# muzishen/IMAGHarmony

Hardware: AMD Instinct MI355X
Metric: 1024^2 SDXL images/sec (30 DDIM steps, PNS N seeds) (higher is better)
Workload: dtype bf16

## Files before the change

### imagharmony_amd/csrc/elementwise.hip

```cpp
#include <algorithm>

#include "imh_common.h"
#include "imh_kernels.h"
#include "imh_philox.h"

namespace imh {

enum : int { EW_TIMESTEP = 0, EW_SILU = 1, EW_CONCAT = 2, EW_CONV_IN = 3, EW_CFG_STEP = 4, EW_CAST_F32 = 5,
             EW_ADD = 6, EW_STEP_SET = 7, EW_CFG_RESCALE = 8, EW_SOFTMAX = 9, EW_ROW_STATS = 10, EW_STEP_ROW = 11, EW_GATHER_ROWS = 12,
             EW_CFG_MSTEP = 13 };

template <typename T>
__global__ void timestep_kernel(const EwParams p) {
    const int dim = p.i0, half = dim >> 1;
    const long long total = p.n * half;
    for (long long i = (long long)blockIdx.x * blockDim.x + threadIdx.x; i < total; i += (long long)gridDim.x * blockDim.x) {
        const int v = (int)(i / half), j = (int)(i % half);
        const float t = p.step ? ((const float*)p.a)[*p.step] : ((const float*)p.a)[v];
        const float f = expf(-9.210340371976184f * (float)j / (float)half);
        const float a = t * f;
        T* y = (T*)p.y + (size_t)v * dim;
        y[j] = from_f32<T>(cosf(a));
        y[half + j] = from_f32<T>(sinf(a));
    }
}

template <typename T>
__global__ void silu_kernel(const EwParams p) {
    typedef typename Vec<T>::v8 v8;
    const long long nv = p.n >> 3;
    for (long long i = (long long)blockIdx.x * blockDim.x + threadIdx.x; i < nv; i += (long long)gridDim.x * blockDim.x) {
        v8 v = ((const v8*)p.a)[i], o;
#pragma unroll
        for (int e = 0; e < 8; ++e) o[e] = from_f32<T>(silu_f(to_f32(v[e])));
        ((v8*)p.y)[i] = o;
    }
}

template <typename T>
__global__ void add_kernel(const EwParams p) {
    typedef typename Vec<T>::v8 v8;
    const long long nv = p.n >> 3;
    for (long long i = (long long)blockIdx.x * blockDim.x + threadIdx.x; i < nv; i += (long long)gridDim.x * blockDim.x) {
        v8 u = ((const v8*)p.a)[i], v = ((const v8*)p.b)[i], o;
#pragma unroll
        for (int e = 0; e < 8; ++e) o[e] = from_f32<T>(to_f32(u[e]) + to_f32(v[e]));
        ((v8*)p.y)[i] = o;
    }
}

template <typename T>
__global__ void concat_kernel(const EwParams p) {
    typedef typename Vec<T>::v8 v8;
    const int c1 = p.i0 >> 3, c2 = p.i1 >> 3, ct = c1 + c2;
    const long long total = p.n * ct;
    for (long long i = (long long)blockIdx.x * blockDim.x + threadIdx.x; i < total; i += (long long)gridDim.x * blockDim.x) {
        const long long pix = i / ct;
        const int c = (int)(i - pix * ct);
        v8 v = c < c1 ? ((const v8*)p.a)[pix * c1 + c] : ((const v8*)p.b)[pix * c2 + (c - c1)];
        ((v8*)p.y)[i] = v;
    }
}

template <typename T, int CIN>
__global__ __launch_bounds__(CIN > 4 ? 512 : 256) void conv_in_kernel(const EwParams p) {
    typedef typename Vec<T>::v8 v8;
    constexpr int KT = CIN * 9;
    extern __shared__ float wl[];
    const int S = p.i0, H = p.i1, W = p.i2, C0 = p.i3, Bout = p.i4;
    const T* w = (const T*)p.w;
    for (int co = threadIdx.x; co < C0; co += blockDim.x) {
#pragma unroll
        for (int k = 0; k < KT; ++k) wl[k * C0 + co] = to_f32(w[co * KT + k]);
    }
    for (int i = threadIdx.x; i < C0; i += blockDim.x) wl[KT * C0 + i] = p.bias ? to_f32(((const T*)p.bias)[i]) : 0.f;
    __syncthreads();
    const int cg = C0 >> 3;
    const float in_scale = p.tab ? p.tab[*p.step] : p.f0;
    const long long total = (long long)Bout * H * W * 8;
    const float* lat = (const float*)p.a;
    for (long long i = (long long)blockIdx.x * blockDim.x + threadIdx.x; i < total; i += (long long)gridDim.x * blockDim.x) {
        const int l8 = (int)(i & 7);
        const long long pix = i >> 3;
        const int x = (int)(pix % W);
        const int y = (int)((pix / W) % H);
        const int b = (int)(pix / ((long long)W * H));
        const float* src = lat + (size_t)(b % S) * 4 * H * W;
        float tap[KT];
#pragma unroll
        for (int ci = 0; ci < 4; ++ci)
#pragma unroll
            for (int ky = 0; ky < 3; ++ky)
#pragma unroll
                for (int kx = 0; kx < 3; ++kx) {
                    const int iy = y + ky - 1, ix = x + kx - 1;
                    const bool in = iy >= 0 && iy < H && ix >= 0 && ix < W;
                    const float v = in ? src[((size_t)ci * H + iy) * W + ix] * in_scale : 0.f;
                    tap[ci * 9 + ky * 3 + kx] = to_f32(from_f32<T>(v));
                }
        if constexpr (CIN > 4) {
            const float* src2 = p.x2 + (size_t)(b % S) * (CIN - 4) * H * W;
#pragma unroll
            for (int ci = 4; ci < CIN; ++ci)
#pragma unroll
                for (int ky = 0; ky < 3; ++ky)
#pragma unroll
                    for (int kx = 0; kx < 3; ++kx) {
                        const int iy = y + ky - 1, ix = x + kx - 1;
                        const bool in = iy >= 0 && iy < H && ix >= 0 && ix < W;
                        const float v = in ? src2[((size_t)(ci - 4) * H + iy) * W + ix] : 0.f;
                        tap[ci * 9 + ky * 3 + kx] = to_f32(from_f32<T>(v));
                    }
        }
        for (int c8 = l8; c8 < cg; c8 += 8) {
            float acc[8];
#pragma unroll
            for (int e = 0; e < 8; ++e) acc[e] = wl[KT * C0 + c8 * 8 + e];
#pragma unroll
            for (int k = 0; k < KT; ++k) {
                const float* wr = wl + k * C0 + c8 * 8;
#pragma unroll
                for (int e = 0; e < 8; ++e) acc[e] += tap[k] * wr[e];
            }
            v8 o;
#pragma unroll
            for (int e = 0; e < 8; ++e) o[e] = from_f32<T>(acc[e]);
            ((v8*)p.y)[pix * cg + c8] = o;
        }
    }
}

template <typename T, bool BLEND>
__global__ void cfg_step_kernel(const EwParams p) {
    const int S = p.i0, HW = p.i1;
    const long long total = (long long)S * HW * 4;
    const T* np_ = (const T*)p.a;
    float* lat = (float*)p.y;
    const float cx = p.tab ? p.tab[*p.step * 2] : p.f0;
    const float ce = p.tab ? p.tab[*p.step * 2 + 1] : p.f1;
    float ba = 0.f, bb = 0.f;
    if constexpr (BLEND) { ba = p.blend_tab[*p.step * 2]; bb = p.blend_tab[*p.step * 2 + 1]; }
    for (long long i = (long long)blockIdx.x * blockDim.x + threadIdx.x; i < total; i += (long long)gridDim.x * blockDim.x) {
        const int pix = (int)(i % HW);
        const int ch = (int)((i / HW) % 4);
        const int s = (int)(i / ((long long)HW * 4));
        if (!BLEND || np_) {
            float eps;
            if (p.i3) {
                const float u = to_f32(np_[((size_t)s * HW + pix) * 4 + ch]);
                const float c = to_f32(np_[((size_t)(S + s) * HW + pix) * 4 + ch]);
                eps = u + p.f2 * (c - u);
            } else {
                eps = to_f32(np_[((size_t)s * HW + pix) * 4 + ch]);
            }
            if (p.w) eps *= ((const float*)p.w)[s];
            if (p.b) ((float*)p.b)[i] = eps;
            lat[i] = cx * lat[i] + ce * eps;
        }
        if constexpr (BLEND) {
            const float m = p.mask[(size_t)(s % p.i4) * HW + pix];
            const float pv = ba * p.x2[i] + bb * p.noise[i];
            lat[i] = (1.0f - m) * pv + m * lat[i];
        }
    }
}

template <typename T, bool BLEND, bool SEEDED = false>
__global__ void cfg_mstep_kernel(const EwParams p) {
    const int S = p.i0, HW = p.i1;
    const long long total = (long long)S * HW * 4;
    const T* np_ = (const T*)p.a;
    float* lat = (float*)p.y;
    float* hist = (float*)p.b;
    const int row = *p.step;
    const float* c = p.tab + (size_t)row * 6;
    const float cx = c[0], ce = c[1], ch = c[2], cn = c[3], hx = c[4], he = c[5];
    const float* z = p.bias ? (const float*)p.bias + (size_t)row * (size_t)total : nullptr;
    float ba = 0.f, bb = 0.f;
    if constexpr (BLEND) { ba = p.blend_tab[row * 2]; bb = p.blend_tab[row * 2 + 1]; }
    if constexpr (SEEDED) {
        const bool gen = cn != 0.f;
        const long long quads = (long long)S * HW;
        for (long long q = (long long)blockIdx.x * blockDim.x + threadIdx.x; q < quads; q += (long long)gridDim.x * blockDim.x) {
            const int s = (int)(q / HW);
            PhiloxNormals zn = {{0.f, 0.f, 0.f, 0.f}};
            if (gen) zn = seeded_normals(p.seeds + (size_t)s * 4, (uint32_t)(q - (long long)s * HW), (uint32_t)row, p.noise_stream);
#pragma unroll
            for (int k = 0; k < 4; ++k) {
                const long long i = q * 4 + k;
                const int pix = (int)(i % HW);
                const int chn = (int)((i / HW) % 4);
                float eps;
                if (p.i3) {
                    const float u = to_f32(np_[((size_t)s * HW + pix) * 4 + chn]);
                    const float cnd = to_f32(np_[((size_t)(S + s) * HW + pix) * 4 + chn]);
                    eps = u + p.f2 * (cnd - u);
                } else {
                    eps = to_f32(np_[((size_t)s * HW + pix) * 4 + chn]);
                }
                if (p.w) eps *= ((const float*)p.w)[s];
                const float x = lat[i];
                float y = cx * x + ce * eps;
                if (hist) {
                    y += ch * hist[i];
                    hist[i] = hx * x + he * eps;
                }
                if (gen) y += cn * zn.z[k];
                if constexpr (BLEND) {
                    const float m = p.mask[(size_t)(s % p.i4) * HW + pix];
                    const float pv = ba * p.x2[i] + bb * p.noise[i];
                    y = (1.0f - m) * pv + m * y;
                }
                lat[i] = y;
            }
        }
        return;
    }
    for (long long i = (long long)blockIdx.x * blockDim.x + threadIdx.x; i < total; i += (long long)gridDim.x * blockDim.x) {
        const int pix = (int)(i % HW);
        const int chn = (int)((i / HW) % 4);
        const int s = (int)(i / ((long long)HW * 4));
        float eps;
        if (p.i3) {
            const float u = to_f32(np_[((size_t)s * HW + pix) * 4 + chn]);
            const float cnd = to_f32(np_[((size_t)(S + s) * HW + pix) * 4 + chn]);
            eps = u + p.f2 * (cnd - u);
        } else {
            eps = to_f32(np_[((size_t)s * HW + pix) * 4 + chn]);
        }
        if (p.w) eps *= ((const float*)p.w)[s];
        const float x = lat[i];
        float y = cx * x + ce * eps;
        if (hist) {
            y += ch * hist[i];
            hist[i] = hx * x + he * eps;
        }
        if (z) y += cn * z[i];
        if constexpr (BLEND) {
            const float m = p.mask[(size_t)(s % p.i4) * HW + pix];
            const float pv = ba * p.x2[i] + bb * p.noise[i];
            y = (1.0f - m) * pv + m * y;
        }
        lat[i] = y;
    }
}

__global__ void randn_seeded_kernel(const RandnParams p) {
    const int HW = p.HW;
    const uint32_t row = p.step ? (uint32_t)*p.step : p.row;
    const long long quads = (long long)p.S * HW;
    for (long long q = (long long)blockIdx.x * blockDim.x + threadIdx.x; q < quads; q += (long long)gridDim.x * blockDim.x) {
        const int s = (int)(q / HW);
        const uint32_t qs = p.quad0 + (uint32_t)(q - (long long)s * HW);
        if (p.raw) {
            const PhiloxWords w = seeded_words(p.seeds + (size_t)s * 4, qs, row, p.noise_stream);
            uint32_t* y = (uint32_t*)p.y + q * 4;
#pragma unroll
            for (int k = 0; k < 4; ++k) y[k] = w.w[k];
        } else {
            const PhiloxNormals n = seeded_normals(p.seeds + (size_t)s * 4, qs, row, p.noise_stream);
            float* y = (float*)p.y + q * 4;
#pragma unroll
            for (int k = 0; k < 4; ++k) y[k] = n.z[k];
        }
    }
}

template <typename T>
__global__ __launch_bounds__(256) void cfg_rescale_kernel(const EwParams p) {
    __shared__ double red[4][256];
    const int S = p.i0, HW = p.i1, s = blockIdx.x;
    const long long n = (long long)HW * 4;
    const T* u = (const T*)p.a + (size_t)s * n;
    const T* c = (const T*)p.a + (size_t)(S + s) * n;
    double st = 0, st2 = 0, sc = 0, sc2 = 0;
    for (long long i = threadIdx.x; i < n; i += 256) {
        const float uu = to_f32(u[i]), cc = to_f32(c[i]);
        const float g = uu + p.f2 * (cc - uu);
        st += cc; st2 += (double)cc * cc; sc += g; sc2 += (double)g * g;
    }
    red[0][threadIdx.x] = st; red[1][threadIdx.x] = st2; red[2][threadIdx.x] = sc; red[3][threadIdx.x] = sc2;
    __syncthreads();
    for (int o = 128; o > 0; o >>= 1) {
        if ((int)threadIdx.x < o)
#pragma unroll
            for (int k = 0; k < 4; ++k) red[k][threadIdx.x] += red[k][threadIdx.x + o];
        __syncthreads();
    }
    if (threadIdx.x == 0) {
        const double N = (double)n;
        const double vt = (red[1][0] - red[0][0] * red[0][0] / N) / (N - 1.0);
        const double vc = (red[3][0] - red[2][0] * red[2][0] / N) / (N - 1.0);
        const double ratio = sqrt(fmax(vt, 0.0)) / sqrt(fmax(vc, 1e-300));
        ((float*)p.y)[s] = (float)(p.f3 * ratio + (1.0 - p.f3));
    }
}

template <typename T>
__global__ __launch_bounds__(256) void softmax_rows_kernel(const EwParams p) {
    __shared__ float red[4];
    const int cols = p.i1, lane = threadIdx.x & 63, wave = threadIdx.x >> 6;
    const float* a = (const float*)p.a + (size_t)blockIdx.x * p.i2;
    T* y = (T*)p.y + (size_t)blockIdx.x * p.i3;
    const float c = p.f0 * 1.4426950408889634f;
    float m = -3.0e38f;
    for (int i = threadIdx.x * 4; i < cols; i += 1024) {
        const f32x4 v = *(const f32x4*)(a + i);
        m = fmaxf(fmaxf(m, fmaxf(v[0], v[1])), fmaxf(v[2], v[3]));
    }
    m = wave_max(m);
    if (lane == 0) red[wave] = m;
    __syncthreads();
    m = fmaxf(fmaxf(red[0], red[1]), fmaxf(red[2], red[3]));
    __syncthreads();
    const float mc = m * c;
    float s = 0.f;
    for (int i = threadIdx.x * 4; i < cols; i += 1024) {
        const f32x4 v = *(const f32x4*)(a + i);
#pragma unroll
        for (int e = 0; e < 4; ++e) s += __builtin_amdgcn_exp2f(v[e] * c - mc);
    }
    s = wave_sum(s);
    if (lane == 0) red[wave] = s;
    __syncthreads();
    const float inv = 1.0f / ((red[0] + red[1]) + (red[2] + red[3]));
    for (int i = threadIdx.x * 4; i < cols; i += 1024) {
        const f32x4 v = *(const f32x4*)(a + i);
        typename Vec<T>::v4 o;
#pragma unroll
        for (int e = 0; e < 4; ++e) o[e] = from_f32<T>(__builtin_amdgcn_exp2f(v[e] * c - mc) * inv);
        *(typename Vec<T>::v4*)(y + i) = o;
    }
}

template <typename T>
__global__ void step_row_kernel(const EwParams p) {
    typedef typename Vec<T>::v8 v8;
    const long long nv = p.n >> 3;
    const v8* src = (const v8*)p.a + (long long)(*p.step) * nv;
    for (long long i = (long long)blockIdx.x * blockDim.x + threadIdx.x; i < nv; i += (long long)gridDim.x * blockDim.x) ((v8*)p.y)[i] = src[i];
}

template <typename T>
__global__ void gather_rows_kernel(const EwParams p) {
    typedef typename Vec<T>::v8 v8;
    const int cv = p.i0 >> 3;
    const long long total = p.n * cv;
    const int* idx = (const int*)p.b;
    for (long long i = (long long)blockIdx.x * blockDim.x + threadIdx.x; i < total; i += (long long)gridDim.x * blockDim.x) {
        const long long r = i / cv;
        const int c = (int)(i - r * cv) * 8;
        const int src = idx[r];
        if ((unsigned)src >= (unsigned)p.i5) continue;
        v8 v = *(const v8*)((const T*)p.a + (size_t)src * p.i1 + c);
        if (p.w) {
            const v8 u = *(const v8*)((const T*)p.w + (size_t)(r % p.i3) * p.i4 + c);
#pragma unroll
            for (int e = 0; e < 8; ++e) v[e] = from_f32<T>(to_f32(v[e]) + to_f32(u[e]));
        }
        *(v8*)((T*)p.y + (size_t)r * p.i2 + c) = v;
    }
}

__global__ void step_set_kernel(int* step, int value, int set) {
    if (threadIdx.x == 0 && blockIdx.x == 0) *step = set ? value : *step + 1;
}

template <typename T>
__global__ void cast_f32_kernel(const EwParams p) {
    for (long long i = (long long)blockIdx.x * blockDim.x + threadIdx.x; i < p.n; i += (long long)gridDim.x * blockDim.x)
        ((float*)p.y)[i] = to_f32(((const T*)p.a)[i]);
}

static inline int grid_for(long long work, int threads) {
    long long g = (work + threads - 1) / threads;
    return (int)(g < 1 ? 1 : (g > 4096 ? 4096 : g));
}

template <typename T>
__global__ __launch_bounds__(256) void row_stats_kernel(const EwParams p) {
    const int lane = threadIdx.x & 63;
    const long long row = (long long)blockIdx.x * 4 + (threadIdx.x >> 6);
    if (row >= p.n) return;
    const T* x = (const T*)p.a + row * p.i1;
    const int C = p.i0;
    float s = 0.f;
    for (int c = lane * 8; c < C; c += 512) {
        const typename Vec<T>::v8 t = *(const typename Vec<T>::v8*)(x + c);
#pragma unroll
        for (int e = 0; e < 8; ++e) s += to_f32(t[e]);
    }
    s = wave_sum(s);
    const float mean = s / (float)C;
    float m2 = 0.f;
    for (int c = lane * 8; c < C; c += 512) {
        const typename Vec<T>::v8 t = *(const typename Vec<T>::v8*)(x + c);
#pragma unroll
        for (int e = 0; e < 8; ++e) { const float d = to_f32(t[e]) - mean; m2 = __builtin_fmaf(d, d, m2); }
    }
    m2 = wave_sum(m2);
    if (lane == 0) { float* y = (float*)p.y + row * 2; y[0] = s; y[1] = m2; }
}

template <typename T>
static int ew_typed(int op, const EwParams& p, hipStream_t stream) {
    switch (op) {
        case EW_TIMESTEP:
            if (p.i0 <= 0 || (p.i0 & 1)) { set_error("timestep: dim must be even"); return IMH_ERR_SHAPE; }
            hipLaunchKernelGGL((timestep_kernel<T>), dim3(grid_for(p.n * (p.i0 >> 1), 256)), dim3(256), 0, stream, p);
            break;
        case EW_SILU:
            if (p.n & 7) { set_error("silu: n must be a multiple of 8"); return IMH_ERR_SHAPE; }
            hipLaunchKernelGGL((silu_kernel<T>), dim3(grid_for(p.n >> 3, 256)), dim3(256), 0, stream, p);
            break;
        case EW_ADD:
            if (p.n & 7) { set_error("add: n must be a multiple of 8"); return IMH_ERR_SHAPE; }
            hipLaunchKernelGGL((add_kernel<T>), dim3(grid_for(p.n >> 3, 256)), dim3(256), 0, stream, p);
            break;
        case EW_CONCAT:
            if ((p.i0 & 7) || (p.i1 & 7)) { set_error("concat: channel counts must be multiples of 8"); return IMH_ERR_SHAPE; }
            hipLaunchKernelGGL((concat_kernel<T>), dim3(grid_for(p.n * ((p.i0 + p.i1) >> 3), 256)), dim3(256), 0, stream, p);
            break;
        case EW_CONV_IN: {
            if (p.i3 & 7) { set_error("conv_in: C0 must be a multiple of 8"); return IMH_ERR_SHAPE; }
            const long long work = (long long)p.i4 * p.i1 * p.i2 * 8;
            if (p.i5 == 9) {
                static DynLdsOnce once;
                const size_t lds = (size_t)(82 * p.i3) * sizeof(float);
                if (!p.x2 || p.i0 <= 0) { set_error("conv_in: 9 input channels need the second source x2 [S, 5, H, W]"); return IMH_ERR_ARG; }
                if (lds > 160 * 1024) { set_error("conv_in: C0 = %d needs %zu bytes of LDS at 9 input channels (160 KiB per workgroup)", p.i3, lds); return IMH_ERR_SHAPE; }
                if (lds > 64 * 1024) once.ensure((const void*)conv_in_kernel<T, 9>, 160 * 1024);
                hipLaunchKernelGGL((conv_in_kernel<T, 9>), dim3(std::min(grid_for(work, 512), lds > 53 * 1024 ? 256 : 768)), dim3(512), lds, stream, p);
                break;
            }
            if (p.i5 != 0 && p.i5 != 4) { set_error("conv_in: %d input channels (4 or 9)", p.i5); return IMH_ERR_ARG; }
            const size_t lds = (size_t)(37 * p.i3) * sizeof(float);
            hipLaunchKernelGGL((conv_in_kernel<T, 4>), dim3(std::min(grid_for(work, 256), 768)), dim3(256), lds, stream, p);
            break;
        }
        case EW_CFG_STEP:
            if (p.mask) {
                if (!p.x2 || !p.noise || !p.blend_tab || !p.step || p.i4 < 1) {
                    set_error("cfg_step: the masked blend needs x2 (image latents), noise, blend_tab, step and i4 = mask batch >= 1");
                    return IMH_ERR_ARG;
                }
                hipLaunchKernelGGL((cfg_step_kernel<T, true>), dim3(grid_for((long long)p.i0 * p.i1 * 4, 256)), dim3(256), 0, stream, p);
                break;
            }
            if (!p.a) { set_error("cfg_step: null noise prediction"); return IMH_ERR_ARG; }
            hipLaunchKernelGGL((cfg_step_kernel<T, false>), dim3(grid_for((long long)p.i0 * p.i1 * 4, 256)), dim3(256), 0, stream, p);
            break;
        case EW_CFG_MSTEP:
            if (!p.a || !p.tab || !p.step || p.i0 <= 0 || p.i1 <= 0) {
                set_error("cfg_mstep: needs the noise prediction, the six-column table, step and S, HW > 0");
                return IMH_ERR_ARG;
            }
            if (p.mask) {
                if (!p.x2 || !p.noise || !p.blend_tab || p.i4 < 1) {
                    set_error("cfg_mstep: the masked blend needs x2 (image latents), noise, blend_tab and i4 = mask batch >= 1");
                    return IMH_ERR_ARG;
                }
                if (p.seeds) hipLaunchKernelGGL((cfg_mstep_kernel<T, true, true>), dim3(grid_for((long long)p.i0 * p.i1, 256)), dim3(256), 0, stream, p);
                else hipLaunchKernelGGL((cfg_mstep_kernel<T, true>), dim3(grid_for((long long)p.i0 * p.i1 * 4, 256)), dim3(256), 0, stream, p);
                break;
            }
            if (p.seeds) hipLaunchKernelGGL((cfg_mstep_kernel<T, false, true>), dim3(grid_for((long long)p.i0 * p.i1, 256)), dim3(256), 0, stream, p);
            else hipLaunchKernelGGL((cfg_mstep_kernel<T, false>), dim3(grid_for((long long)p.i0 * p.i1 * 4, 256)), dim3(256), 0, stream, p);
            break;
        case EW_CFG_RESCALE:
            if (p.i0 <= 0 || p.i1 <= 0) { set_error("cfg_rescale: empty problem"); return IMH_ERR_SHAPE; }
            hipLaunchKernelGGL((cfg_rescale_kernel<T>), dim3(p.i0), dim3(256), 0, stream, p);
            break;
        case EW_SOFTMAX:
            if (p.i0 <= 0 || p.i1 <= 0 || (p.i1 & 3) || (p.i2 & 3) || (p.i3 & 3) || p.f0 <= 0.f) {
                set_error("softmax: rows=%d cols=%d ld=%d/%d (cols and lds must be multiples of 4, scale > 0)", p.i0, p.i1, p.i2, p.i3);
                return IMH_ERR_SHAPE;
            }
            hipLaunchKernelGGL((softmax_rows_kernel<T>), dim3(p.i0), dim3(256), 0, stream, p);
            break;
        case EW_CAST_F32:
            hipLaunchKernelGGL((cast_f32_kernel<T>), dim3(grid_for(p.n, 256)), dim3(256), 0, stream, p);
            break;
        case EW_ROW_STATS:
            if (p.n <= 0 || p.i0 <= 0 || (p.i0 & 7) || (p.i1 & 7) || !p.a) { set_error("row_stats: rows=%lld C=%d ld=%d (C and ld must be multiples of 8)", p.n, p.i0, p.i1); return IMH_ERR_SHAPE; }
            hipLaunchKernelGGL((row_stats_kernel<T>), dim3((unsigned)((p.n + 3) / 4)), dim3(256), 0, stream, p);
            break;
        case EW_STEP_ROW:
            if (p.n <= 0 || (p.n & 7) || !p.a || !p.step) { set_error("step_row: n=%lld must be a positive multiple of 8, a and step non-null", p.n); return IMH_ERR_ARG; }
            hipLaunchKernelGGL((step_row_kernel<T>), dim3(grid_for(p.n >> 3, 256)), dim3(256), 0, stream, p);
            break;
        case EW_GATHER_ROWS:
            if (!p.a || !p.b || p.n <= 0 || p.i0 <= 0 || (p.i0 & 7) || p.i1 < p.i0 || (p.i1 & 7) || p.i2 < p.i0 || (p.i2 & 7) || p.i5 <= 0 ||
                (p.w && (p.i3 <= 0 || p.i4 < p.i0 || (p.i4 & 7)))) {
                set_error("gather_rows: n=%lld C=%d ld=%d/%d table rows=%d add rows=%d ld=%d (table, idx non-null; C and the row strides multiples of 8, "
                          "strides >= C; table rows > 0; with add: rows > 0)", p.n, p.i0, p.i1, p.i2, p.i5, p.i3, p.i4);
                return IMH_ERR_SHAPE;
            }
            if ((((uintptr_t)p.a | (uintptr_t)p.y | (uintptr_t)p.w) & 15) || ((uintptr_t)p.b & 3)) {
                set_error("gather_rows: table / add / y must be 16-byte aligned, idx 4-byte aligned"); return IMH_ERR_ARG;
            }
            hipLaunchKernelGGL((gather_rows_kernel<T>), dim3(grid_for(p.n * (p.i0 >> 3), 256)), dim3(256), 0, stream, p);
            break;
        case EW_STEP_SET:
            hipLaunchKernelGGL(step_set_kernel, dim3(1), dim3(64), 0, stream, (int*)p.y, p.i0, p.i1);
            break;
        default:
            set_error("elementwise: unknown op %d", op);
            return IMH_ERR_ARG;
    }
    return check_launch("elementwise");
}

int randn_seeded_launch(const RandnParams& p, hipStream_t stream) {
    hipLaunchKernelGGL(randn_seeded_kernel, dim3(grid_for((long long)p.S * p.HW, 256)), dim3(256), 0, stream, p);
    return check_launch("randn_seeded");
}

int randn_seeded_host(const RandnParams& p) {
    const uint32_t row = p.step ? (uint32_t)*p.step : p.row;
    for (int s = 0; s < p.S; ++s)
        for (int q = 0; q < p.HW; ++q) {
            const size_t o = ((size_t)s * p.HW + q) * 4;
            if (p.raw) {
                const PhiloxWords w = seeded_words(p.seeds + (size_t)s * 4, p.quad0 + (uint32_t)q, row, p.noise_stream);
                for (int k = 0; k < 4; ++k) ((uint32_t*)p.y)[o + k] = w.w[k];
            } else {
                const PhiloxNormals n = seeded_normals(p.seeds + (size_t)s * 4, p.quad0 + (uint32_t)q, row, p.noise_stream);
                for (int k = 0; k < 4; ++k) ((float*)p.y)[o + k] = n.z[k];
            }
        }
    return IMH_OK;
}

int ew_launch(int op, const EwParams& p, int dtype, hipStream_t stream) {
    if (dtype == IMH_DT_BF16) return ew_typed<bf16_t>(op, p, stream);
    if (dtype == IMH_DT_F16) return ew_typed<f16_t>(op, p, stream);
    set_error("elementwise: unknown dtype %d", dtype);
    return IMH_ERR_DTYPE;
}

}
```

### imagharmony_amd/csrc/norm.hip

```cpp
#include "imh_common.h"
#include "imh_kernels.h"
#include "imh_gntable.h"
#include <algorithm>

namespace imh {

constexpr int GN_THREADS = 512;
constexpr int GN_ELEMS_PER_BLOCK = 8192;

static inline int gn_nblk(int HW, int C) {
    long long e = (long long)HW * C;
    int n = (int)((e + GN_ELEMS_PER_BLOCK - 1) / GN_ELEMS_PER_BLOCK);
    return n < 1 ? 1 : (n > 256 ? 256 : n);
}
static inline int gn_sub(int C, int groups) {
    const int cpg = C / groups;
    return (cpg % 10 == 0) ? 10 : cpg;
}
int groupnorm_stats_blocks(int HW, int C) { return gn_nblk(HW, C); }
int groupnorm_stats_sub(int C, int groups) { return gn_sub(C, groups); }

size_t groupnorm_workspace_bytes(int B, int HW, int C, int groups) {
    const size_t part = (size_t)B * gn_nblk(HW, C) * (C / gn_sub(C, groups)) * 2 * sizeof(float);
    return ((part + 255) & ~(size_t)255) + (size_t)B * C * 2 * sizeof(float);
}

__device__ __forceinline__ void chan_merge(float& n, float& s, float& m2, const float nb, const float sb, const float mb) {
    if (nb <= 0.f) return;
    if (n <= 0.f) { n = nb; s = sb; m2 = mb; return; }
    const float nn = n + nb;
    const float d = sb / nb - s / n;
    m2 = m2 + mb + d * d * (n * nb / nn);
    s += sb;
    n = nn;
}

template <typename T, typename Load>
__device__ __forceinline__ void gn_stats_block(const int C, const int HW, const int nblk, const int sub, float* partial, float* lds, Load load) {
    typedef typename Vec<T>::v8 v8;
    const int CL = C >> 3;
    const int P = max(1, GN_THREADS / CL);
    float* ls = lds;
    float* lm = lds + P * C;
    float* ln = lds + 2 * P * C;
    const int b = blockIdx.y, blk = blockIdx.x;
    const int ppb = (HW + nblk - 1) / nblk;
    const int start = blk * ppb, end = min(HW, start + ppb);
    const int t = threadIdx.x;
    if (t < CL * P) {
        const int cl = t % CL, pl = t / CL;
        float s[8], q[8], pv[8];
#pragma unroll
        for (int e = 0; e < 8; ++e) { s[e] = 0.f; q[e] = 0.f; pv[e] = 0.f; }
        int cnt = 0;
        for (int pix = start + pl; pix < end; pix += P) {
            const v8 v = load(b, pix, cl);
            if (cnt == 0) {
#pragma unroll
                for (int e = 0; e < 8; ++e) pv[e] = to_f32(v[e]);
            }
#pragma unroll
            for (int e = 0; e < 8; ++e) { const float f = to_f32(v[e]) - pv[e]; s[e] += f; q[e] = __builtin_fmaf(f, f, q[e]); }
            ++cnt;
        }
        const float n = (float)cnt;
#pragma unroll
        for (int e = 0; e < 8; ++e) {
            ls[pl * C + cl * 8 + e] = __builtin_fmaf(n, pv[e], s[e]);
            lm[pl * C + cl * 8 + e] = cnt ? fmaxf(q[e] - s[e] * s[e] / n, 0.f) : 0.f;
        }
        if (cl == 0) ln[pl] = n;
    }
    __syncthreads();
    const int nsub = C / sub;
    for (int j = t; j < nsub; j += GN_THREADS) {
        float n = 0.f, s = 0.f, m2 = 0.f;
        for (int pl = 0; pl < P; ++pl) {
            const float np = ln[pl];
            for (int c = j * sub; c < (j + 1) * sub; ++c) chan_merge(n, s, m2, np, ls[pl * C + c], lm[pl * C + c]);
        }
        float* o = partial + (((size_t)b * nblk + blk) * nsub + j) * 2;
        o[0] = s; o[1] = m2;
    }
}

template <typename T>
__global__ __launch_bounds__(GN_THREADS) void gn_stats_kernel(const NormParams p, int nblk, int sub) {
    typedef typename Vec<T>::v8 v8;
    extern __shared__ float lds[];
    const T* x = (const T*)p.x;
    const int C = p.C, HW = p.HW;
    gn_stats_block<T>(C, HW, nblk, sub, p.partial, lds, [&](int b, int pix, int cl) -> v8 {
        return *(const v8*)(x + ((size_t)b * HW + pix) * C + cl * 8);
    });
}

template <typename T, bool STATS>
__global__ __launch_bounds__(GN_THREADS) void control_add_kernel(const ControlAddParams p, int nblk) {
    typedef typename Vec<T>::v8 v8;
    extern __shared__ float lds[];
    const T* x = (const T*)p.x;
    const T* r = (const T*)p.r;
    T* y = (T*)p.y;
    const int C = p.C, HW = p.HW, Br = p.Br;
    const float g = p.tab ? __fmul_rn(p.scale, p.tab[*p.step]) : p.scale;
    auto one = [&](int b, int pix, int cl) -> v8 {
        const size_t off = ((size_t)b * HW + pix) * C + cl * 8;
        const v8 xv = *(const v8*)(x + off);
        const v8 rv = *(const v8*)(r + ((size_t)(b % Br) * HW + pix) * C + cl * 8);
        v8 o;
#pragma unroll
        for (int e = 0; e < 8; ++e) o[e] = from_f32<T>(__fadd_rn(to_f32(xv[e]), __fmul_rn(g, to_f32(rv[e]))));
        *(v8*)(y + off) = o;
        return o;
    };
    if constexpr (STATS) {
        gn_stats_block<T>(C, HW, nblk, p.sub, p.partial, lds, one);
    } else {
        const int CL = C >> 3;
        const int P = max(1, GN_THREADS / CL);
        const int ppb = (HW + nblk - 1) / nblk;
        const int start = blockIdx.x * ppb, end = min(HW, start + ppb);
        const int t = threadIdx.x;
        if (t < CL * P)
            for (int pix = start + t / CL; pix < end; pix += P) one(blockIdx.y, pix, t % CL);
    }
}

int control_add_launch(const ControlAddParams& p, int dtype, hipStream_t stream) {
    if (p.C <= 0 || p.C % 8 || (p.C >> 3) > GN_THREADS || p.B <= 0 || p.B > 65535 || p.HW <= 0 || p.Br <= 0 || p.B % p.Br) {
        set_error("control_add: unsupported B=%d Br=%d HW=%d C=%d (C a multiple of 8 up to %d, Br a divisor of B)", p.B, p.Br, p.HW, p.C, GN_THREADS * 8);
        return IMH_ERR_SHAPE;
    }
    if (dtype != IMH_DT_BF16 && dtype != IMH_DT_F16) { set_error("control_add: unknown dtype %d", dtype); return IMH_ERR_DTYPE; }
    if (p.partial && (p.sub <= 0 || p.C % p.sub)) { set_error("control_add: sub-run width %d does not divide C=%d", p.sub, p.C); return IMH_ERR_ARG; }
    const int nblk = gn_nblk(p.HW, p.C);
    dim3 grid(nblk, p.B);
    if (p.partial) {
        const int P = std::max(1, GN_THREADS / (p.C >> 3));
        const size_t lds = (2 * (size_t)p.C * P + P) * sizeof(float);
        if (dtype == IMH_DT_BF16) hipLaunchKernelGGL((control_add_kernel<bf16_t, true>), grid, dim3(GN_THREADS), lds, stream, p, nblk);
        else hipLaunchKernelGGL((control_add_kernel<f16_t, true>), grid, dim3(GN_THREADS), lds, stream, p, nblk);
    } else {
        if (dtype == IMH_DT_BF16) hipLaunchKernelGGL((control_add_kernel<bf16_t, false>), grid, dim3(GN_THREADS), 0, stream, p, nblk);
        else hipLaunchKernelGGL((control_add_kernel<f16_t, false>), grid, dim3(GN_THREADS), 0, stream, p, nblk);
    }
    return check_launch("control_add_kernel");
}

static inline GnTabSrc gn_src_of(const NormParams& p) {
    GnTabSrc g;
    g.partial = p.partial; g.partial2 = p.partial2; g.gamma = p.gamma; g.beta = p.beta; g.eps = p.eps;
    g.groups = p.groups; g.C = p.C; g.C1 = p.partial2 ? p.C1 : p.C; g.HW = p.HW;
    g.nblk = p.nblk; g.sub = p.sub; g.npart = p.npart; g.nblk2 = p.nblk2; g.sub2 = p.sub2; g.npart2 = p.npart2;
    g.dtype_f16 = p.dtype_f16;
    return g;
}
__global__ __launch_bounds__(256) void gn_table_kernel(const GnTabSrc g, float* table) {
    const int b = blockIdx.y, t = threadIdx.x;
    const int gg = blockIdx.x * (256 / GN_GL) + t / GN_GL;
    if (gg >= g.groups) return;
    GnRows r;
    gn_rows_fetch(g, gg, t & (GN_GL - 1), r);
    float mean, rstd;
    gn_group_stats(g, b, gg, t & (GN_GL - 1), mean, rstd);
    gn_group_rows(g, gg, t & (GN_GL - 1), mean, rstd, r, table + (size_t)b * g.C * 2);
}

template <typename T, bool OWN>
__global__ __launch_bounds__(GN_THREADS) void gn_apply_kernel(const NormParams p, int nblk, const GnTabSrc g) {
    typedef typename Vec<T>::v8 v8;
    extern __shared__ __attribute__((aligned(16))) float gn_lds_tab[];
    tail_prefetch(p.pf_ptr, p.pf_bytes, blockIdx.x + gridDim.x * blockIdx.y, gridDim.x * gridDim.y, threadIdx.x, GN_THREADS);
    const int C = p.C, CL = C >> 3;
    const int P = max(1, GN_THREADS / CL);
    const int b = blockIdx.y, blk = blockIdx.x;
    const int ppb = (p.HW + nblk - 1) / nblk;
    const int start = blk * ppb, end = min(p.HW, start + ppb);
    const int t = threadIdx.x;
    if constexpr (OWN) {
        gn_table_of_sample(g, b, gn_lds_tab, t / GN_GL, GN_THREADS / GN_GL, t & 63);
        __syncthreads();
    }
    if (t < CL * P) {
        const int cl = t % CL, pl = t / CL;
        float sc[8], sh[8];
        {
            const f32x4* tb = OWN ? (const f32x4*)(gn_lds_tab + (size_t)cl * 8 * 2) : (const f32x4*)(p.table + ((size_t)b * C + cl * 8) * 2);
#pragma unroll
            for (int e = 0; e < 4; ++e) { const f32x4 v = tb[e]; sc[2 * e] = v[0]; sh[2 * e] = v[1]; sc[2 * e + 1] = v[2]; sh[2 * e + 1] = v[3]; }
        }
        const T* x = (const T*)p.x + ((size_t)b * p.HW) * C + cl * 8;
        T* y = (T*)p.y + ((size_t)b * p.HW) * C + cl * 8;
        auto one = [&](const v8& v, size_t off) {
            v8 o;
#pragma unroll
            for (int e = 0; e < 8; ++e) {
                float f = __builtin_fmaf(to_f32(v[e]), sc[e], sh[e]);
                if (p.silu) f = silu_f(f);
                o[e] = from_f32<T>(f);
            }
            *(v8*)(y + off) = o;
        };
        int pix = start + pl;
        for (; pix + 3 * P < end; pix += 4 * P) {
            const size_t o0 = (size_t)pix * C, o1 = (size_t)(pix + P) * C, o2 = (size_t)(pix + 2 * P) * C, o3 = (size_t)(pix + 3 * P) * C;
            v8 v0 = *(const v8*)(x + o0), v1 = *(const v8*)(x + o1), v2 = *(const v8*)(x + o2), v3 = *(const v8*)(x + o3);
            one(v0, o0); one(v1, o1); one(v2, o2); one(v3, o3);
        }
        for (; pix < end; pix += P) one(*(const v8*)(x + (size_t)pix * C), (size_t)pix * C);
    }
}

int groupnorm_launch(const NormParams& p0, int dtype, hipStream_t stream) {
    NormParams p = p0;
    if (p.C % 8 || p.groups <= 0 || p.groups > 64 || p.C % p.groups || (p.C >> 3) > GN_THREADS || p.B <= 0 || p.HW <= 0) {
        set_error("groupnorm: unsupported B=%d HW=%d C=%d groups=%d", p.B, p.HW, p.C, p.groups);
        return IMH_ERR_SHAPE;
    }
    if (dtype != IMH_DT_BF16 && dtype != IMH_DT_F16) { set_error("groupnorm: unknown dtype %d", dtype); return IMH_ERR_DTYPE; }
    p.dtype_f16 = dtype == IMH_DT_F16;
    const int nblk = gn_nblk(p.HW, p.C);
    const int mode = p.mode;
    if (mode < 0 || mode > 4) { set_error("groupnorm: unknown mode %d", mode); return IMH_ERR_ARG; }
    const int cpg = p.C / p.groups;
    if (mode == 4) {
        if (!p.partial2) p.C1 = p.C;
        const GnTabSrc g = gn_src_of(p);
        if (!p.x || !p.y || !gn_src_ok(g)) {
            set_error("groupnorm table+apply: needs x, y and partials whose sub-runs tile the groups (C=%d groups=%d C1=%d sub=%d/%d nblk=%d/%d), eps > 0",
                      p.C, p.groups, p.C1, p.sub, p.sub2, p.nblk, p.nblk2);
            return IMH_ERR_ARG;
        }
        const size_t lds = (size_t)p.C * 2 * sizeof(float);
        dim3 grid(nblk, p.B);
        if (dtype == IMH_DT_BF16) hipLaunchKernelGGL((gn_apply_kernel<bf16_t, true>), grid, dim3(GN_THREADS), lds, stream, p, nblk, g);
        else hipLaunchKernelGGL((gn_apply_kernel<f16_t, true>), grid, dim3(GN_THREADS), lds, stream, p, nblk, g);
        return check_launch("groupnorm table+apply");
    }
    if (mode == 0 || mode == 1) {
        if (!p.x || !p.partial) { set_error("groupnorm: statistics need x and a partial / workspace buffer"); return p.x ? IMH_ERR_WORKSPACE : IMH_ERR_ARG; }
        const int sub = mode == 0 ? gn_sub(p.C, p.groups) : p.sub;
        if (sub <= 0 || p.C % sub || (mode == 0 && cpg % sub)) { set_error("groupnorm: sub-run width %d does not divide C=%d", sub, p.C); return IMH_ERR_ARG; }
        const int P = std::max(1, GN_THREADS / (p.C >> 3));
        const size_t lds = (2 * (size_t)p.C * P + P) * sizeof(float);
        dim3 grid(nblk, p.B);
        if (dtype == IMH_DT_BF16) hipLaunchKernelGGL((gn_stats_kernel<bf16_t>), grid, dim3(GN_THREADS), lds, stream, p, nblk, sub);
        else hipLaunchKernelGGL((gn_stats_kernel<f16_t>), grid, dim3(GN_THREADS), lds, stream, p, nblk, sub);
        if (mode == 1) return check_launch("gn_stats_kernel");
        const size_t part = (size_t)p.B * nblk * (p.C / sub) * 2 * sizeof(float);
        p.table = (float*)((unsigned char*)p.partial + ((part + 255) & ~(size_t)255));
        p.partial2 = nullptr; p.C1 = p.C; p.sub = sub; p.nblk = nblk; p.npart = 0;
    }
    if (mode == 0 || mode == 2) {
        if (!p.partial || !p.table) { set_error("groupnorm: the table step needs partials and a table buffer"); return IMH_ERR_ARG; }
        if (!p.partial2) p.C1 = p.C;
        const GnTabSrc g = gn_src_of(p);
        if (!gn_src_ok(g)) {
            set_error("groupnorm table: sub-runs must tile the groups (C=%d groups=%d C1=%d sub=%d/%d nblk=%d/%d) and eps > 0", p.C, p.groups, p.C1, p.sub, p.sub2, p.nblk, p.nblk2);
            return IMH_ERR_ARG;
        }
        hipLaunchKernelGGL(gn_table_kernel, dim3((p.groups * GN_GL + 255) / 256, p.B), dim3(256), 0, stream, g, p.table);
        if (mode == 2) return check_launch("gn_table_kernel");
    }
    if (!p.x || !p.y || !p.table) { set_error("groupnorm: apply needs x, y and a table"); return IMH_ERR_ARG; }
    dim3 grid(nblk, p.B);
    if (dtype == IMH_DT_BF16) hipLaunchKernelGGL((gn_apply_kernel<bf16_t, false>), grid, dim3(GN_THREADS), 0, stream, p, nblk, GnTabSrc{});
    else hipLaunchKernelGGL((gn_apply_kernel<f16_t, false>), grid, dim3(GN_THREADS), 0, stream, p, nblk, GnTabSrc{});
    return check_launch("groupnorm");
}

template <typename T, int NCH, int ROWS>
__global__ __launch_bounds__(256) void ln_kernel(const NormParams p) {
    typedef typename Vec<T>::v8 v8;
    const int lane = threadIdx.x & 63;
    tail_prefetch(p.pf_ptr, p.pf_bytes, blockIdx.x, gridDim.x, threadIdx.x, 256);
    const int row0 = (blockIdx.x * 4 + (threadIdx.x >> 6)) * ROWS;
    if (row0 >= p.rows) return;
    const int C = p.C, CL = C >> 3;
    float v[ROWS][NCH][8];
    float s[ROWS];
#pragma unroll
    for (int r = 0; r < ROWS; ++r) {
        const int row = min(row0 + r, p.rows - 1);
        const T* x = (const T*)p.x + (size_t)row * C;
        s[r] = 0.f;
#pragma unroll
        for (int k = 0; k < NCH; ++k) {
            const int ch = lane + k * 64;
            if (ch < CL) {
                v8 t = *(const v8*)(x + ch * 8);
#pragma unroll
                for (int e = 0; e < 8; ++e) { v[r][k][e] = to_f32(t[e]); s[r] += v[r][k][e]; }
            } else {
#pragma unroll
                for (int e = 0; e < 8; ++e) v[r][k][e] = 0.f;
            }
        }
    }
    const T* ga = (const T*)p.gamma;
    const T* be = (const T*)p.beta;
#pragma unroll
    for (int r = 0; r < ROWS; ++r) {
        const float mean = wave_sum(s[r]) / C;
        float q = 0.f;
#pragma unroll
        for (int k = 0; k < NCH; ++k) {
            const int ch = lane + k * 64;
            if (ch < CL) {
#pragma unroll
                for (int e = 0; e < 8; ++e) { const float d = v[r][k][e] - mean; q += d * d; }
            }
        }
        const float rstd = rsqrtf(wave_sum(q) / C + p.eps);
        if (row0 + r >= p.rows) continue;
        T* y = (T*)p.y + (size_t)(row0 + r) * C;
#pragma unroll
        for (int k = 0; k < NCH; ++k) {
            const int ch = lane + k * 64;
            if (ch < CL) {
                v8 g8, b8, o;
                if (ga) g8 = *(const v8*)(ga + ch * 8);
                if (be) b8 = *(const v8*)(be + ch * 8);
#pragma unroll
                for (int e = 0; e < 8; ++e) {
                    float f = (v[r][k][e] - mean) * rstd;
                    if (ga) f *= to_f32(g8[e]);
                    if (be) f += to_f32(b8[e]);
                    o[e] = from_f32<T>(f);
                }
                *(v8*)(y + ch * 8) = o;
            }
        }
    }
}

template <typename T>
static int ln_typed(const NormParams& p, hipStream_t stream) {
    const int cl = p.C >> 3;
    if (cl <= 128) hipLaunchKernelGGL((ln_kernel<T, 2, 1>), dim3((p.rows + 3) / 4), dim3(256), 0, stream, p);
    else if (cl <= 256) hipLaunchKernelGGL((ln_kernel<T, 4, 1>), dim3((p.rows + 3) / 4), dim3(256), 0, stream, p);
    else hipLaunchKernelGGL((ln_kernel<T, 8, 1>), dim3((p.rows + 3) / 4), dim3(256), 0, stream, p);
    return check_launch("ln_kernel");
}

int layernorm_launch(const NormParams& p, int dtype, hipStream_t stream) {
    if (p.C % 8 || p.C > 4096 || p.rows <= 0) { set_error("layernorm: unsupported C=%d rows=%d", p.C, p.rows); return IMH_ERR_SHAPE; }
    if (dtype == IMH_DT_BF16) return ln_typed<bf16_t>(p, stream);
    if (dtype == IMH_DT_F16) return ln_typed<f16_t>(p, stream);
    set_error("layernorm: unknown dtype %d", dtype);
    return IMH_ERR_DTYPE;
}

}
```

Baseline: 1.710.

## Rework conv_in weight staging, dedupe batch outputs, restructure groupnorm stats and apply

conv_in now loads weights with coalesced unrolled reads into a padded LDS layout to avoid bank conflicts. It computes each unique seed sample once and writes the result to every duplicated batch slot. Groupnorm statistics are rewritten to use unrolled loads and a parallel, fixed-order merge of per-lane partial sums and M2 terms instead of the serial Chan merge. The fused table+apply kernel prefetches inputs before the table build and uses fewer, larger blocks. These changes raise LDS use and add more complex indexing, with some risk of numerical differences and lower occupancy.

```diff
diff --git a/imagharmony_amd/csrc/elementwise.hip b/imagharmony_amd/csrc/elementwise.hip
--- a/imagharmony_amd/csrc/elementwise.hip
+++ b/imagharmony_amd/csrc/elementwise.hip
@@ -62,6 +62,8 @@
     }
 }
 
+__host__ __device__ __forceinline__ int conv_in_row_stride(int C0) { return C0 + 1; }
+static inline size_t conv_in_lds_bytes(int C0, int cin) { return ((size_t)cin * 9 * conv_in_row_stride(C0) + C0) * sizeof(float); }
 template <typename T, int CIN>
 __global__ __launch_bounds__(CIN > 4 ? 512 : 256) void conv_in_kernel(const EwParams p) {
     typedef typename Vec<T>::v8 v8;
@@ -69,15 +71,27 @@
     extern __shared__ float wl[];
     const int S = p.i0, H = p.i1, W = p.i2, C0 = p.i3, Bout = p.i4;
     const T* w = (const T*)p.w;
-    for (int co = threadIdx.x; co < C0; co += blockDim.x) {
-#pragma unroll
-        for (int k = 0; k < KT; ++k) wl[k * C0 + co] = to_f32(w[co * KT + k]);
-    }
-    for (int i = threadIdx.x; i < C0; i += blockDim.x) wl[KT * C0 + i] = p.bias ? to_f32(((const T*)p.bias)[i]) : 0.f;
+    const int CS = conv_in_row_stride(C0);
+    {
+        const int nw = C0 * KT;
+        constexpr int UW = 8;
+        for (int i0 = threadIdx.x; i0 < nw; i0 += UW * blockDim.x) {
+            T v[UW];
+#pragma unroll
+            for (int u = 0; u < UW; ++u) { const int i = i0 + u * blockDim.x; if (i < nw) v[u] = w[i]; }
+#pragma unroll
+            for (int u = 0; u < UW; ++u) {
+                const int i = i0 + u * blockDim.x;
+                if (i < nw) { const int co = i / KT; wl[(i - co * KT) * CS + co] = to_f32(v[u]); }
+            }
+        }
+    }
+    for (int i = threadIdx.x; i < C0; i += blockDim.x) wl[KT * CS + i] = p.bias ? to_f32(((const T*)p.bias)[i]) : 0.f;
     __syncthreads();
     const int cg = C0 >> 3;
     const float in_scale = p.tab ? p.tab[*p.step] : p.f0;
-    const long long total = (long long)Bout * H * W * 8;
+    const long long total = (long long)min(S, Bout) * H * W * 8;
+    const size_t bstride = (size_t)S * H * W * cg;
     const float* lat = (const float*)p.a;
     for (long long i = (long long)blockIdx.x * blockDim.x + threadIdx.x; i < total; i += (long long)gridDim.x * blockDim.x) {
         const int l8 = (int)(i & 7);
@@ -85,7 +99,7 @@
         const int x = (int)(pix % W);
         const int y = (int)((pix / W) % H);
         const int b = (int)(pix / ((long long)W * H));
-        const float* src = lat + (size_t)(b % S) * 4 * H * W;
+        const float* src = lat + (size_t)b * 4 * H * W;
         float tap[KT];
 #pragma unroll
         for (int ci = 0; ci < 4; ++ci)
@@ -99,7 +113,7 @@
                     tap[ci * 9 + ky * 3 + kx] = to_f32(from_f32<T>(v));
                 }
         if constexpr (CIN > 4) {
-            const float* src2 = p.x2 + (size_t)(b % S) * (CIN - 4) * H * W;
+            const float* src2 = p.x2 + (size_t)b * (CIN - 4) * H * W;
 #pragma unroll
             for (int ci = 4; ci < CIN; ++ci)
 #pragma unroll
@@ -115,17 +129,18 @@
         for (int c8 = l8; c8 < cg; c8 += 8) {
             float acc[8];
 #pragma unroll
-            for (int e = 0; e < 8; ++e) acc[e] = wl[KT * C0 + c8 * 8 + e];
+            for (int e = 0; e < 8; ++e) acc[e] = wl[KT * CS + c8 * 8 + e];
 #pragma unroll
             for (int k = 0; k < KT; ++k) {
-                const float* wr = wl + k * C0 + c8 * 8;
+                const float* wr = wl + k * CS + c8 * 8;
 #pragma unroll
                 for (int e = 0; e < 8; ++e) acc[e] += tap[k] * wr[e];
             }
             v8 o;
 #pragma unroll
             for (int e = 0; e < 8; ++e) o[e] = from_f32<T>(acc[e]);
-            ((v8*)p.y)[pix * cg + c8] = o;
+            v8* dst = (v8*)p.y + pix * cg + c8;
+            for (int bo = b; bo < Bout; bo += S, dst += bstride) *dst = o;
         }
     }
 }
@@ -423,10 +438,10 @@
             break;
         case EW_CONV_IN: {
             if (p.i3 & 7) { set_error("conv_in: C0 must be a multiple of 8"); return IMH_ERR_SHAPE; }
-            const long long work = (long long)p.i4 * p.i1 * p.i2 * 8;
+            const long long work = (long long)std::min(p.i0 > 0 ? p.i0 : p.i4, p.i4) * p.i1 * p.i2 * 8;
             if (p.i5 == 9) {
                 static DynLdsOnce once;
-                const size_t lds = (size_t)(82 * p.i3) * sizeof(float);
+                const size_t lds = conv_in_lds_bytes(p.i3, 9);
                 if (!p.x2 || p.i0 <= 0) { set_error("conv_in: 9 input channels need the second source x2 [S, 5, H, W]"); return IMH_ERR_ARG; }
                 if (lds > 160 * 1024) { set_error("conv_in: C0 = %d needs %zu bytes of LDS at 9 input channels (160 KiB per workgroup)", p.i3, lds); return IMH_ERR_SHAPE; }
                 if (lds > 64 * 1024) once.ensure((const void*)conv_in_kernel<T, 9>, 160 * 1024);
@@ -434,7 +449,7 @@
                 break;
             }
             if (p.i5 != 0 && p.i5 != 4) { set_error("conv_in: %d input channels (4 or 9)", p.i5); return IMH_ERR_ARG; }
-            const size_t lds = (size_t)(37 * p.i3) * sizeof(float);
+            const size_t lds = conv_in_lds_bytes(p.i3, 4);
             hipLaunchKernelGGL((conv_in_kernel<T, 4>), dim3(std::min(grid_for(work, 256), 768)), dim3(256), lds, stream, p);
             break;
         }
diff --git a/imagharmony_amd/csrc/norm.hip b/imagharmony_amd/csrc/norm.hip
--- a/imagharmony_amd/csrc/norm.hip
+++ b/imagharmony_amd/csrc/norm.hip
@@ -25,27 +25,28 @@
     return ((part + 255) & ~(size_t)255) + (size_t)B * C * 2 * sizeof(float);
 }
 
-__device__ __forceinline__ void chan_merge(float& n, float& s, float& m2, const float nb, const float sb, const float mb) {
-    if (nb <= 0.f) return;
-    if (n <= 0.f) { n = nb; s = sb; m2 = mb; return; }
-    const float nn = n + nb;
-    const float d = sb / nb - s / n;
-    m2 = m2 + mb + d * d * (n * nb / nn);
-    s += sb;
-    n = nn;
-}
-
+constexpr int GN_LU = 8;
+constexpr int GN_MU = 8;
+static inline size_t gn_stats_lds_bytes(int C, int sub) {
+    const int K = std::max(1, GN_THREADS / (C >> 3)) * sub;
+    return (3 * (size_t)(C / sub) * (K | 1) + 2 * (size_t)K) * sizeof(float);
+}
 template <typename T, typename Load>
 __device__ __forceinline__ void gn_stats_block(const int C, const int HW, const int nblk, const int sub, float* partial, float* lds, Load load) {
     typedef typename Vec<T>::v8 v8;
     const int CL = C >> 3;
     const int P = max(1, GN_THREADS / CL);
+    const int K = P * sub, KS = K | 1;
+    const int nsub = C / sub;
     float* ls = lds;
-    float* lm = lds + P * C;
-    float* ln = lds + 2 * P * C;
+    float* lm = ls + nsub * KS;
+    float* la = lm + nsub * KS;
+    float* lnb = la + nsub * KS;
+    float* lw = lnb + K;
     const int b = blockIdx.y, blk = blockIdx.x;
     const int ppb = (HW + nblk - 1) / nblk;
     const int start = blk * ppb, end = min(HW, start + ppb);
+    const int Ke = min(P, max(end - start, 0)) * sub;
     const int t = threadIdx.x;
     if (t < CL * P) {
         const int cl = t % CL, pl = t / CL;
@@ -53,34 +54,101 @@
 #pragma unroll
         for (int e = 0; e < 8; ++e) { s[e] = 0.f; q[e] = 0.f; pv[e] = 0.f; }
         int cnt = 0;
-        for (int pix = start + pl; pix < end; pix += P) {
-            const v8 v = load(b, pix, cl);
+        for (int pix = start + pl; pix < end; pix += GN_LU * P) {
+            v8 v[GN_LU];
+#pragma unroll
+            for (int u = 0; u < GN_LU; ++u)
+                if (pix + u * P < end) v[u] = load(b, pix + u * P, cl);
             if (cnt == 0) {
 #pragma unroll
-                for (int e = 0; e < 8; ++e) pv[e] = to_f32(v[e]);
-            }
-#pragma unroll
-            for (int e = 0; e < 8; ++e) { const float f = to_f32(v[e]) - pv[e]; s[e] += f; q[e] = __builtin_fmaf(f, f, q[e]); }
-            ++cnt;
-        }
-        const float n = (float)cnt;
-#pragma unroll
-        for (int e = 0; e < 8; ++e) {
-            ls[pl * C + cl * 8 + e] = __builtin_fmaf(n, pv[e], s[e]);
-            lm[pl * C + cl * 8 + e] = cnt ? fmaxf(q[e] - s[e] * s[e] / n, 0.f) : 0.f;
-        }
-        if (cl == 0) ln[pl] = n;
+                for (int e = 0; e < 8; ++e) pv[e] = to_f32(v[0][e]);
+            }
+#pragma unroll
+            for (int u = 0; u < GN_LU; ++u)
+                if (pix + u * P < end) {
+#pragma unroll
+                    for (int e = 0; e < 8; ++e) { const float f = to_f32(v[u][e]) - pv[e]; s[e] += f; q[e] = __builtin_fmaf(f, f, q[e]); }
+                    ++cnt;
+                }
+        }
+        if (cnt) {
+            const float n = (float)cnt;
+            int j = cl * 8 / sub, ci = cl * 8 - j * sub;
+#pragma unroll
+            for (int e = 0; e < 8; ++e) {
+                const int i = j * KS + pl * sub + ci;
+                const float sum = __builtin_fmaf(n, pv[e], s[e]);
+                ls[i] = sum;
+                lm[i] = fmaxf(q[e] - s[e] * s[e] / n, 0.f);
+                la[i] = sum / n;
+                if (++ci == sub) { ci = 0; ++j; }
+            }
+        }
+    }
+    for (int k = GN_THREADS - 1 - t; k < Ke; k += GN_THREADS) {
+        const int pl = k / sub, ci = k - pl * sub;
+        float n = 0.f;
+        for (int q = 0; q < pl; ++q) {
+            const float nq = (float)((end - start - q + P - 1) / P);
+            for (int c = 0; c < sub; ++c) n += nq;
+        }
+        const float nb = (float)((end - start - pl + P - 1) / P);
+        for (int c = 0; c < ci; ++c) n += nb;
+        lnb[k] = n;
+        lw[k] = __fmul_rn(n, nb) / (n + nb);
     }
     __syncthreads();
-    const int nsub = C / sub;
     for (int j = t; j < nsub; j += GN_THREADS) {
-        float n = 0.f, s = 0.f, m2 = 0.f;
-        for (int pl = 0; pl < P; ++pl) {
-            const float np = ln[pl];
-            for (int c = j * sub; c < (j + 1) * sub; ++c) chan_merge(n, s, m2, np, ls[pl * C + c], lm[pl * C + c]);
-        }
-        float* o = partial + (((size_t)b * nblk + blk) * nsub + j) * 2;
-        o[0] = s; o[1] = m2;
+        float* row = ls + j * KS;
+        float s = 0.f;
+        float cur[GN_MU], nxt[GN_MU];
+#pragma unroll
+        for (int u = 0; u < GN_MU; ++u) cur[u] = row[min(u, max(Ke - 1, 0))];
+        for (int k0 = 0; k0 < Ke; k0 += GN_MU) {
+#pragma unroll
+            for (int u = 0; u < GN_MU; ++u) nxt[u] = row[min(k0 + GN_MU + u, Ke - 1)];
+#pragma unroll
+            for (int u = 0; u < GN_MU; ++u)
+                if (k0 + u < Ke) {
+                    row[k0 + u] = s;
+                    s = k0 + u == 0 ? cur[u] : __fadd_rn(s, cur[u]);
+                }
+#pragma unroll
+            for (int u = 0; u < GN_MU; ++u) cur[u] = nxt[u];
+        }
+        partial[(((size_t)b * nblk + blk) * nsub + j) * 2] = s;
+    }
+    __syncthreads();
+    {
+        int j = t / KS, k = t - j * KS;
+        const int dj = GN_THREADS / KS, dk = GN_THREADS - dj * KS;
+        for (int i = t; i < nsub * KS; i += GN_THREADS) {
+            if (k > 0 && k < Ke) {
+                const float d = la[i] - ls[i] / lnb[k];
+                la[i] = __fmul_rn(__fmul_rn(d, d), lw[k]);
+            }
+            j += dj; k += dk;
+            if (k >= KS) { k -= KS; ++j; }
+        }
+    }
+    __syncthreads();
+    for (int j = t; j < nsub; j += GN_THREADS) {
+        const float* rm = lm + j * KS;
+        const float* ra = la + j * KS;
+        float m2 = 0.f;
+        float cm[GN_MU], ca[GN_MU], nm[GN_MU], na[GN_MU];
+#pragma unroll
+        for (int u = 0; u < GN_MU; ++u) { cm[u] = rm[min(u, max(Ke - 1, 0))]; ca[u] = ra[min(u, max(Ke - 1, 0))]; }
+        for (int k0 = 0; k0 < Ke; k0 += GN_MU) {
+#pragma unroll
+            for (int u = 0; u < GN_MU; ++u) { nm[u] = rm[min(k0 + GN_MU + u, Ke - 1)]; na[u] = ra[min(k0 + GN_MU + u, Ke - 1)]; }
+#pragma unroll
+            for (int u = 0; u < GN_MU; ++u)
+                if (k0 + u < Ke) m2 = k0 + u == 0 ? cm[u] : __fadd_rn(__fadd_rn(m2, cm[u]), ca[u]);
+#pragma unroll
+            for (int u = 0; u < GN_MU; ++u) { cm[u] = nm[u]; ca[u] = na[u]; }
+        }
+        partial[(((size_t)b * nblk + blk) * nsub + j) * 2 + 1] = m2;
     }
 }
 
@@ -137,10 +205,15 @@
     const int nblk = gn_nblk(p.HW, p.C);
     dim3 grid(nblk, p.B);
     if (p.partial) {
-        const int P = std::max(1, GN_THREADS / (p.C >> 3));
-        const size_t lds = (2 * (size_t)p.C * P + P) * sizeof(float);
-        if (dtype == IMH_DT_BF16) hipLaunchKernelGGL((control_add_kernel<bf16_t, true>), grid, dim3(GN_THREADS), lds, stream, p, nblk);
-        else hipLaunchKernelGGL((control_add_kernel<f16_t, true>), grid, dim3(GN_THREADS), lds, stream, p, nblk);
+        const size_t lds = gn_stats_lds_bytes(p.C, p.sub);
+        static DynLdsOnce once[2];
+        if (dtype == IMH_DT_BF16) {
+            if (lds > 64 * 1024) once[0].ensure((const void*)control_add_kernel<bf16_t, true>, 160 * 1024);
+            hipLaunchKernelGGL((control_add_kernel<bf16_t, true>), grid, dim3(GN_THREADS), lds, stream, p, nblk);
+        } else {
+            if (lds > 64 * 1024) once[1].ensure((const void*)control_add_kernel<f16_t, true>, 160 * 1024);
+            hipLaunchKernelGGL((control_add_kernel<f16_t, true>), grid, dim3(GN_THREADS), lds, stream, p, nblk);
+        }
     } else {
         if (dtype == IMH_DT_BF16) hipLaunchKernelGGL((control_add_kernel<bf16_t, false>), grid, dim3(GN_THREADS), 0, stream, p, nblk);
         else hipLaunchKernelGGL((control_add_kernel<f16_t, false>), grid, dim3(GN_THREADS), 0, stream, p, nblk);
@@ -167,6 +240,7 @@
     gn_group_rows(g, gg, t & (GN_GL - 1), mean, rstd, r, table + (size_t)b * g.C * 2);
 }
 
+constexpr int GN_APPLY_FAT = 2;
 template <typename T, bool OWN>
 __global__ __launch_bounds__(GN_THREADS) void gn_apply_kernel(const NormParams p, int nblk, const GnTabSrc g) {
     typedef typename Vec<T>::v8 v8;
@@ -178,12 +252,20 @@
     const int ppb = (p.HW + nblk - 1) / nblk;
     const int start = blk * ppb, end = min(p.HW, start + ppb);
     const int t = threadIdx.x;
+    const int cl = t % CL, pl = t / CL;
+    constexpr int AU = 8;
+    v8 pre[AU];
     if constexpr (OWN) {
+        if (t < CL * P) {
+            const T* xp = (const T*)p.x + ((size_t)b * p.HW) * C + cl * 8;
+#pragma unroll
+            for (int u = 0; u < AU; ++u)
+                if (start + pl + u * P < end) pre[u] = *(const v8*)(xp + (size_t)(start + pl + u * P) * C);
+        }
         gn_table_of_sample(g, b, gn_lds_tab, t / GN_GL, GN_THREADS / GN_GL, t & 63);
         __syncthreads();
     }
     if (t < CL * P) {
-        const int cl = t % CL, pl = t / CL;
         float sc[8], sh[8];
         {
             const f32x4* tb = OWN ? (const f32x4*)(gn_lds_tab + (size_t)cl * 8 * 2) : (const f32x4*)(p.table + ((size_t)b * C + cl * 8) * 2);
@@ -203,12 +285,26 @@
             *(v8*)(y + off) = o;
         };
         int pix = start + pl;
-        for (; pix + 3 * P < end; pix += 4 * P) {
-            const size_t o0 = (size_t)pix * C, o1 = (size_t)(pix + P) * C, o2 = (size_t)(pix + 2 * P) * C, o3 = (size_t)(pix + 3 * P) * C;
-            v8 v0 = *(const v8*)(x + o0), v1 = *(const v8*)(x + o1), v2 = *(const v8*)(x + o2), v3 = *(const v8*)(x + o3);
-            one(v0, o0); one(v1, o1); one(v2, o2); one(v3, o3);
-        }
-        for (; pix < end; pix += P) one(*(const v8*)(x + (size_t)pix * C), (size_t)pix * C);
+        if constexpr (OWN) {
+            for (; pix < end; pix += AU * P) {
+                v8 nxt[AU];
+#pragma unroll
+                for (int u = 0; u < AU; ++u)
+                    if (pix + (AU + u) * P < end) nxt[u] = *(const v8*)(x + (size_t)(pix + (AU + u) * P) * C);
+#pragma unroll
+                for (int u = 0; u < AU; ++u)
+                    if (pix + u * P < end) one(pre[u], (size_t)(pix + u * P) * C);
+#pragma unroll
+                for (int u = 0; u < AU; ++u) pre[u] = nxt[u];
+            }
+        } else {
+            for (; pix + 3 * P < end; pix += 4 * P) {
+                const size_t o0 = (size_t)pix * C, o1 = (size_t)(pix + P) * C, o2 = (size_t)(pix + 2 * P) * C, o3 = (size_t)(pix + 3 * P) * C;
+                v8 v0 = *(const v8*)(x + o0), v1 = *(const v8*)(x + o1), v2 = *(const v8*)(x + o2), v3 = *(const v8*)(x + o3);
+                one(v0, o0); one(v1, o1); one(v2, o2); one(v3, o3);
+            }
+            for (; pix < end; pix += P) one(*(const v8*)(x + (size_t)pix * C), (size_t)pix * C);
+        }
     }
 }
 
@@ -233,20 +329,26 @@
             return IMH_ERR_ARG;
         }
         const size_t lds = (size_t)p.C * 2 * sizeof(float);
-        dim3 grid(nblk, p.B);
-        if (dtype == IMH_DT_BF16) hipLaunchKernelGGL((gn_apply_kernel<bf16_t, true>), grid, dim3(GN_THREADS), lds, stream, p, nblk, g);
-        else hipLaunchKernelGGL((gn_apply_kernel<f16_t, true>), grid, dim3(GN_THREADS), lds, stream, p, nblk, g);
+        const int ablk = (nblk + GN_APPLY_FAT - 1) / GN_APPLY_FAT;
+        dim3 grid(ablk, p.B);
+        if (dtype == IMH_DT_BF16) hipLaunchKernelGGL((gn_apply_kernel<bf16_t, true>), grid, dim3(GN_THREADS), lds, stream, p, ablk, g);
+        else hipLaunchKernelGGL((gn_apply_kernel<f16_t, true>), grid, dim3(GN_THREADS), lds, stream, p, ablk, g);
         return check_launch("groupnorm table+apply");
     }
     if (mode == 0 || mode == 1) {
         if (!p.x || !p.partial) { set_error("groupnorm: statistics need x and a partial / workspace buffer"); return p.x ? IMH_ERR_WORKSPACE : IMH_ERR_ARG; }
         const int sub = mode == 0 ? gn_sub(p.C, p.groups) : p.sub;
         if (sub <= 0 || p.C % sub || (mode == 0 && cpg % sub)) { set_error("groupnorm: sub-run width %d does not divide C=%d", sub, p.C); return IMH_ERR_ARG; }
-        const int P = std::max(1, GN_THREADS / (p.C >> 3));
-        const size_t lds = (2 * (size_t)p.C * P + P) * sizeof(float);
+        const size_t lds = gn_stats_lds_bytes(p.C, sub);
+        static DynLdsOnce once[2];
         dim3 grid(nblk, p.B);
-        if (dtype == IMH_DT_BF16) hipLaunchKernelGGL((gn_stats_kernel<bf16_t>), grid, dim3(GN_THREADS), lds, stream, p, nblk, sub);
-        else hipLaunchKernelGGL((gn_stats_kernel<f16_t>), grid, dim3(GN_THREADS), lds, stream, p, nblk, sub);
+        if (dtype == IMH_DT_BF16) {
+            if (lds > 64 * 1024) once[0].ensure((const void*)gn_stats_kernel<bf16_t>, 160 * 1024);
+            hipLaunchKernelGGL((gn_stats_kernel<bf16_t>), grid, dim3(GN_THREADS), lds, stream, p, nblk, sub);
+        } else {
+            if (lds > 64 * 1024) once[1].ensure((const void*)gn_stats_kernel<f16_t>, 160 * 1024);
+            hipLaunchKernelGGL((gn_stats_kernel<f16_t>), grid, dim3(GN_THREADS), lds, stream, p, nblk, sub);
+        }
         if (mode == 1) return check_launch("gn_stats_kernel");
         const size_t part = (size_t)p.B * nblk * (p.C / sub) * 2 * sizeof(float);
         p.table = (float*)((unsigned char*)p.partial + ((part + 255) & ~(size_t)255));
```

Result: no change. 1.713 (median of 6 runs) (+0.2%).
